# loli/medpy

Measured on AMD Instinct MI355X. Metric: Mvoxels/s graph-cut (build+solve), 512^3 6-conn; fraction of HBM roofline, higher is better.
Workload: dtype f64

## Files before the change

medpy_amd/csrc/mgc_kernels.hip:

```cpp
#include <hip/hip_runtime.h>
#include <rccl/rccl.h>

#include <dlfcn.h>

#include <math.h>
#include <stdarg.h>
#include <stdio.h>
#include <stdlib.h>
#include <string.h>

#include <algorithm>
#include <map>
#include <string>
#include <mutex>
#include <thread>
#include <vector>

#include "../../include/medpy_hip.h"
#include "mgc_tile_ops.inl"
#include "mgc_tile_ops26.inl"
#include "mgc_wave_ops.inl"
#include "mgc_wave_ops26.inl"
#include "mgc_dt_ops.inl"
#include "mgc_brick_ops.inl"
// ... 737 lines not shown
                }
            } else if (mode == 1) {
                take = (L.status[tile] & (MGC_ST_EXCESS | MGC_ST_ALLINF)) == MGC_ST_EXCESS;
            } else if (mode == 3) {
                take = (L.status[tile] & MGC_ST_SINK) != 0;
            } else {
                take = (L.status[tile] & MGC_ST_SUSPECT) != 0;
            }
        }
        const unsigned long long m = __ballot(take);
        if (m) {
            int pos = 0;
            const int sh = (int)(blockIdx.x & (unsigned)(L.nshard - 1));
            if ((threadIdx.x & 63) == 0) pos = atomicAdd(mgc_counter(L, cnt, sh), __popcll(m));
            pos = __shfl(pos, 0);
            if (take) L.list[list][(int64_t)sh * L.shard_cap + pos + __popcll(m & ((1ull << (threadIdx.x & 63)) - 1ull))] = tile;
        }
    }
}

__global__ __launch_bounds__(MGC_TV) void k_relabel_first_list(MgcLattice L, int list, int cnt, uint32_t epoch, int next_list)
{
    __shared__ MgcTileShared S;
    GpuBlock x(S);
    MgcListView view;
    const int n = mgc_list_view(L, cnt, view);
    if (blockIdx.x == 0 && threadIdx.x == 0 && n) atomicAdd(&L.count[9], n);
    for (int i = blockIdx.x; i < n; i += gridDim.x) {
        x.new_tile();
        mgc_relabel_tile(x, L, mgc_list_at(L, list, view, i), epoch, next_list, true);
        __syncthreads();
    }
}

__global__ __launch_bounds__(256) void k_absorb_w(MgcLattice L, int list, int cnt, int clear_cnt)
{
    __shared__ MgcWaveShared S;
    GpuWave w(S);
    mgc_clear_counter(L, clear_cnt);
    MgcListView view;
    const int n = mgc_list_view(L, cnt, view);
    for (int i = (int)blockIdx.x * 4 + (int)(threadIdx.x >> 6); i < n; i += (int)gridDim.x * 4) {
        w.new_tile();
        mgcw_absorb_tile(w, L, __builtin_amdgcn_readfirstlane(mgc_list_at(L, list, view, i)));
    }
}

__global__ __launch_bounds__(MGC_TV) void k_absorb_list(MgcLattice L, int list, int cnt, int clear_cnt)
{
    mgc_clear_counter(L, clear_cnt);
    __shared__ MgcTileShared S;
    GpuBlock x(S);
    MgcListView view;
    const int n = mgc_list_view(L, cnt, view);
    for (int i = blockIdx.x; i < n; i += gridDim.x) {
        x.new_tile();
        mgc_absorb_tile(x, L, mgc_list_at(L, list, view, i));
        __syncthreads();
    }
}

__global__ __launch_bounds__(MGC_TV) void k_activate_list(MgcLattice L, int list, int cnt, uint32_t phase)
{
    __shared__ MgcTileShared S;
    GpuBlock x(S);
    MgcListView view;
    const int n = mgc_list_view(L, cnt, view);
    for (int i = blockIdx.x; i < n; i += gridDim.x) {
        x.new_tile();
        mgc_activate_tile(x, L, mgc_list_at(L, list, view, i), phase);
        __syncthreads();
    }
}

template <int AXIS, bool BWD, int SEED, int FINAL>
__global__ __launch_bounds__(256) void k_dt_scan(MgcLattice L, const void* in, void* out, int c_min, int32_t* hout, const uint16_t* carry_in, uint16_t* carry_out, int carry_plane)
{
    __shared__ MgcWaveShared S;
    GpuWave w(S);
    const int n = mgc_dt_lines<AXIS>(L);
    for (int line = (int)blockIdx.x * 4 + (int)(threadIdx.x >> 6); line < n; line += (int)gridDim.x * 4) {
        w.new_tile();
        mgc_dt_scan_line<AXIS, BWD, SEED, FINAL>(w, L, __builtin_amdgcn_readfirstlane(line), in, out, c_min, hout, carry_in, carry_out, carry_plane);
    }
}

__global__ __launch_bounds__(256) void k_shadow_sync(MgcLattice L)
{
    __shared__ MgcWaveShared S;
    GpuWave w(S);
    const int T = L.gy * L.gx;
    for (int i = (int)blockIdx.x * 4 + (int)(threadIdx.x >> 6); i < 2 * T; i += (int)gridDim.x * 4) {
        w.new_tile();
        mgc_shadow_sync_tile(w, L, i / T, __builtin_amdgcn_readfirstlane(i % T), L.height);
    }
}

__global__ __launch_bounds__(256) void k_dt_finish(MgcLattice L)
{
    __shared__ MgcWaveShared S;
    GpuWave w(S);
    if (blockIdx.x == 0 && threadIdx.x == 0) atomicAdd(&L.count[9], L.ntiles);
    for (int tile = (int)blockIdx.x * 4 + (int)(threadIdx.x >> 6); tile < L.ntiles; tile += (int)gridDim.x * 4) {
        w.new_tile();
        mgc_dt_finish_tile(w, L, __builtin_amdgcn_readfirstlane(tile));
    }
}

__global__ __launch_bounds__(256) void k_dt_cmin(MgcLattice L)
{
    __shared__ MgcWaveShared S;
    GpuWave w(S);
    for (int tile = (int)blockIdx.x * 4 + (int)(threadIdx.x >> 6); tile < L.ntiles; tile += (int)gridDim.x * 4) {
        w.new_tile();
        mgc_dt_cmin_tile(w, L, __builtin_amdgcn_readfirstlane(tile));
    }
}

__global__ __launch_bounds__(256) void k_dt_lower(MgcLattice L, const uint16_t* ds, int c_min)
{
    __shared__ MgcWaveShared S;
    GpuWave w(S);
    for (int tile = (int)blockIdx.x * 4 + (int)(threadIdx.x >> 6); tile < L.ntiles; tile += (int)gridDim.x * 4) {
        w.new_tile();
        mgc_dt_lower_tile(w, L, __builtin_amdgcn_readfirstlane(tile), ds, c_min);
    }
}

__global__ __launch_bounds__(256) void k_source_open(MgcLattice L)
{
    __shared__ MgcWaveShared S;
    GpuWave w(S);
    for (int tile = (int)blockIdx.x * 4 + (int)(threadIdx.x >> 6); tile < L.ntiles; tile += (int)gridDim.x * 4) {
        w.new_tile();
        mgc_source_open_tile(w, L, __builtin_amdgcn_readfirstlane(tile));
    }
}

__global__ __launch_bounds__(256) void k_activate_w(MgcLattice L, int list, int cnt, uint32_t phase, int exact_max, int clear_cnt)
{
    mgc_clear_counter(L, clear_cnt);
    __shared__ MgcWaveShared S;
    GpuWave w(S);
    MgcListView view;
    const int n = mgc_list_view(L, cnt, view);
    if (n <= exact_max) {
        for (int i = (int)blockIdx.x * 4 + (int)(threadIdx.x >> 6); i < n; i += (int)gridDim.x * 4) {
            w.new_tile();
            mgcw_activate_tile(w, L, __builtin_amdgcn_readfirstlane(mgc_list_at(L, list, view, i)), phase, true);
        }
        return;
    }
    const int sh = (int)(blockIdx.x & (unsigned)(L.nshard - 1)), lane = (int)(threadIdx.x & 63);
    for (int base = (int)blockIdx.x * 256; base < n; base += (int)gridDim.x * 256) {
        const int i = base + (int)threadIdx.x;
        const bool take = i < n;
        const int tile = take ? mgc_list_at(L, list, view, i) : 0;
        int tz, ty, tx;
        mgc_tile_coords(L, tile, tz, ty, tx);
        const uint32_t target = phase + ((mgc_tile_colour(L, tz, ty, tx) ^ (int)(phase & 1u)) & 1);
        for (uint32_t tg = phase; tg <= phase + 1; ++tg) {
            const unsigned long long m = __ballot(take && target == tg);
            if (!m) continue;
            int pos = 0;
            if (lane == 0) pos = atomicAdd(mgc_counter(L, (int)(tg & 3u), sh), __popcll(m));
            pos = __shfl(pos, 0);
// ... 1274 lines not shown

struct MgcRoctx {
    bool tried = false;
    int (*push)(const char*) = nullptr;
    int (*pop)() = nullptr;
    void resolve()
    {
        tried = true;
        const char* on = getenv("MEDPY_HIP_ROCTX");
        if (!on || !*on || *on == '0') return;
        for (const char* n : {"librocprofiler-sdk-roctx.so.1", "librocprofiler-sdk-roctx.so", "libroctx64.so.4", "libroctx64.so"}) {
            void* dl = dlopen(n, RTLD_NOW | RTLD_GLOBAL);
            if (!dl) continue;
            *(void**)(&push) = dlsym(dl, "roctxRangePushA");
            *(void**)(&pop) = dlsym(dl, "roctxRangePop");
            if (push && pop) return;
            push = nullptr; pop = nullptr;
        }
    }
};
static MgcRoctx g_roctx;
static inline void mgc_range_push(const char* name)
{
    if (!g_roctx.tried) g_roctx.resolve();
    if (g_roctx.push) (void)g_roctx.push(name);
}
static inline void mgc_range_pop()
{
    if (g_roctx.pop) (void)g_roctx.pop();
}
struct MgcRange {
    explicit MgcRange(const char* name) { mgc_range_push(name); }
    ~MgcRange() { mgc_range_pop(); }
};
static std::string g_create_error;

struct mgc_graph {
    int device = 0;
    int ndim = 0;
    int64_t shape[3] = {1, 1, 1};
    int64_t nvox = 0;
    hipStream_t stream = nullptr;
    hipEvent_t ev[4] = {nullptr, nullptr, nullptr, nullptr};
    std::vector<hipEvent_t> ev_pool;
    struct OpSpan { int a, b, kind; };
    std::vector<hipEvent_t> op_ev;
    std::vector<OpSpan> op_spans;
    MgcLattice L{};
    void* d_image = nullptr; int img_dtype = 0; int term = MGC_TERM_NONE; double sigma = 0; double spacing[3] = {1, 1, 1};
    int has_spacing = 0;
    void* d_prob = nullptr; int prob_dtype = 0; double alpha = 0;
    void* d_lut = nullptr; int lut_n = 0;
    uint8_t* d_fg = nullptr; uint8_t* d_bg = nullptr;
    double* d_tr_in = nullptr; double flow_const_in = 0;
    MgcBuildArgs build_args{};
    int64_t n_edges = 0, n_runs = 0; int64_t* d_eslot = nullptr; double* d_eval = nullptr; int64_t* d_erun = nullptr;
    bool range_set = false; double range[3] = {0, 0, 0};
    bool edges_applied = false;
    std::map<const void*, size_t> buf_cap;
    uint8_t* d_tsum = nullptr;
    uint8_t* d_tflags = nullptr;
    double* d_tr0 = nullptr; double* d_part = nullptr; double* d_part2 = nullptr; double* d_scalar = nullptr; uint8_t* d_labels = nullptr;
    int32_t* h_count = nullptr;
    double* h_scalar = nullptr;
    uint8_t* h_labels = nullptr; bool labels_on_host = false;
    bool built = false, solved = false;
    bool unconverged = false;
    bool labels_valid = false;
    void* d_vout = nullptr;
    uint16_t* d_dt16 = nullptr;
    uint16_t* d_ds16 = nullptr;
    int32_t* d_hexact = nullptr;
    bool radial_on = false;
    int radial_cycle_no = 0;
    bool all_residual = false;
    int exact_sink_tiles = 1;
    int sink_tiles = 0;
    int wall_tiles = 0;
    int radial_min_walls = 16;
    int sink_sweeps = 8;
    int use_bricks = 0;
    bool brick_mode = false;
    int use_dt = 1;
    int rank = 0, nranks = 1;
    int64_t plane0 = 0, plane1 = 0, own0 = 0, own1 = 0;
    int64_t gd0 = 0;
    uint16_t* d_carry[2] = {nullptr, nullptr};
    uint16_t* d_carry_in[2] = {nullptr, nullptr};
    uint16_t* dt_cur = nullptr;
    void* d_halo = nullptr; int64_t halo_cap = 0;
    ncclComm_t comm = nullptr; void* d_xchg[4] = {nullptr, nullptr, nullptr, nullptr}; int64_t xchg_cap = 0;
    int64_t* d_cnt64 = nullptr;
    double flow_const = 0.0, flow = 0.0;
    MgcSolveParams params = mgc_default_params();
    int grid_cap = 4096;
    int grid26_dis = 16384;
    int wave_kernels = 9;
    int wave_grid_dis = 0, wave_grid_rel = 0;
    int tk_dis = MGC_CNT_TICKET_DIS, tk_rel = MGC_CNT_TICKET_REL;
    int est_phase_tiles = 1 << 30;
    int sweeps_sparse26 = 5;
    int wave_grid26 = 0;
    bool rounds_set = false, sparse26_set = false, wave_set = false;
    bool w26_auto = false;
    int prepush = 1;
    int w26_passes = 2, w26_raises = 1, w26_flags = 0;
    int activate_exact_max = 4096;
    int wave_stagger = 0;
    int repeat_steps = 1;
    int repeat_min_tiles = 0;
    int repeat_flood_min_tiles = 200000;
    bool repeat_now = false;
    int wave_min_tiles = 512;
    uint32_t zero_mask = 0;
    int filt[2] = {0, 0};
    int pending_zero = -1;
    int use_filters = 3;
    mgc_stats stats{};
    int64_t device_bytes = 0;
    std::string err;
    bool timing = true;
    int timing_stride = 7;
    uint32_t timing_offset = 0;
};

static int mgc_fail(mgc_handle h, int code, const char* fmt, ...)
{
    char buf[512];
    va_list ap;
    va_start(ap, fmt);
    vsnprintf(buf, sizeof(buf), fmt, ap);
    va_end(ap);
    if (h) h->err = buf;
    else g_create_error = buf;
    return code;
}

#define MGC_HIP(h, call)                                                                                       \
    do {                                                                                                       \
        hipError_t e_ = (call);                                                                                \
        if (e_ != hipSuccess)                                                                                  \
            return mgc_fail(h, e_ == hipErrorOutOfMemory ? MGC_ERR_OOM : MGC_ERR_HIP, "%s failed: %s (%s:%d)", \
                            #call, hipGetErrorString(e_), __FILE__, __LINE__);                                 \
    } while (0)


#define MGC_POOL_MIN ((size_t)1 << 20)
struct MgcPool {
    std::mutex lock;
    std::multimap<size_t, void*> idle[16];
    std::map<void*, std::pair<size_t, int>> live;
    size_t idle_bytes[16] = {0};
    long long budget[16];
    long long hits = 0, misses = 0;
    MgcPool() { for (auto& b : budget) b = -1; }
    long long budget_of(int dev)
    {
        if (budget[dev] < 0) {
            const char* e = getenv("MEDPY_HIP_POOL_MB");
            if (e && *e) budget[dev] = atoll(e) << 20;
            else {
                size_t f = 0, t = 0;
                budget[dev] = hipMemGetInfo(&f, &t) == hipSuccess ? (long long)(t / 8) : 0;
            }
        }
        return budget[dev];
// ... 85 lines not shown
    void fill_heights_inf()
    {
        flush_zero();
        h->labels_valid = true;
        check(hipMemsetAsync(h->L.height, 0x3f, (size_t)h->L.ntiles * MGC_TV * sizeof(int32_t), h->stream));
        hipLaunchKernelGGL(k_status_or, dim3((h->L.ntiles + 255) / 256), dim3(256), 0, h->stream, h->L, (uint32_t)MGC_ST_ALLINF, (uint32_t)MGC_ST_SETTLED);
        for (int sd = 0; sd < 2; ++sd)
            if (h->L.hshadow[sd]) check(hipMemsetAsync(h->L.hshadow[sd], 0x3f, (size_t)h->L.gy * h->L.gx * MGC_TF * sizeof(int32_t), h->stream));
    }
    void flush_zero()
    {
        if (h->pending_zero >= 0) h->zero_mask |= 1u << h->pending_zero;
        h->pending_zero = -1;
        if (h->zero_mask) {
            hipLaunchKernelGGL(k_zero_counts, dim3(1), dim3(MGC_NCOUNT * MGC_NSHARD), 0, h->stream, h->L, h->zero_mask);
            check(hipGetLastError());
        }
        h->zero_mask = 0;
    }
    void zero_count(int i)
    {
        if (i == last_discharged) { flush_zero(); h->pending_zero = i; last_discharged = -1; return; }
        if (h->pending_zero >= 0) { h->zero_mask |= 1u << h->pending_zero; h->pending_zero = -1; }
        h->zero_mask |= 1u << i;
    }
    void read_counts(int* out)
    {
        flush_zero();
        check(hipMemcpyAsync(h->h_count, h->L.count, MGC_NCOUNT * (1 + MGC_NSHARD) * sizeof(int32_t), hipMemcpyDeviceToHost, h->stream));
        check(hipStreamSynchronize(h->stream));
        mgc_fold_counts(h);
        memcpy(out, h->h_count, MGC_NCOUNT * sizeof(int32_t));
        readbacks++;
        if (!FULL) {
            int m = out[6] / 2;
            for (int i = 0; i < 4; ++i) m = out[i] > m ? out[i] : m;
            h->est_phase_tiles = m;
        } else {
            int m = out[MGC26_CNT_ACTIVE] / 8;
            for (int i = 0; i < MGC26_NLIST; ++i) m = out[i] > m ? out[i] : m;
            h->est_phase_tiles = m;
        }
    }
    int filter_grid() const { const int g = (h->L.ntiles + 255) / 256; return g < 1024 ? g : 1024; }
    int fslot(int which) const { return which == 0 ? (h->filt[0] ? MGC_CNT_FILTER_B : MGC_CNT_FILTER) : (h->filt[1] ? MGC_CNT_FILTER_ACT_B : MGC_CNT_FILTER_ACT); }
    int fnext(int which) const { return which == 0 ? (h->filt[0] ? MGC_CNT_FILTER : MGC_CNT_FILTER_B) : (h->filt[1] ? MGC_CNT_FILTER_ACT : MGC_CNT_FILTER_ACT_B); }
    void filter_done(int which, bool consumer_cleared_next)
    {
        if (!consumer_cleared_next) zero_count(fnext(which));
        h->filt[which] ^= 1;
    }
    void absorb_all()
    {
        flush_zero();
        if constexpr (FULL) return;
        else if (!(h->use_filters & 1)) { hipLaunchKernelGGL(k_absorb, dim3(grid(h->L.ntiles)), dim3(MGC_TV), 0, h->stream, h->L); check(hipGetLastError()); }
        else {
            flush_zero();
            hipLaunchKernelGGL(k_filter, dim3(filter_grid()), dim3(256), 0, h->stream, h->L, 0, 6, fslot(0));
            if (h->wave_kernels & 1) hipLaunchKernelGGL(k_absorb_w, dim3(grid((h->L.ntiles + 3) / 4)), dim3(256), 0, h->stream, h->L, 6, fslot(0), fnext(0));
            else hipLaunchKernelGGL(k_absorb_list, dim3(grid(h->L.ntiles)), dim3(MGC_TV), 0, h->stream, h->L, 6, fslot(0), fnext(0));
            filter_done(0, true);
            check(hipGetLastError());
        }
    }
    void relabel_all(uint32_t epoch, int next)
    {
        flush_zero();
        h->brick_mode = false;
        const int id = time_begin(1);
        if constexpr (FULL) hipLaunchKernelGGL(k26_relabel_all, dim3(grid(h->L.ntiles)), dim3(MGC_TV), 0, h->stream, h->L, epoch, next);
        else if (!(h->use_filters & 1)) hipLaunchKernelGGL(k_relabel_all, dim3(grid(h->L.ntiles)), dim3(MGC_TV), 0, h->stream, h->L, epoch, next);
        else {
            flush_zero();
            hipLaunchKernelGGL(k_filter, dim3(filter_grid()), dim3(256), 0, h->stream, h->L, 3, 6, fslot(0));
            if (h->wave_kernels & 8) { hipLaunchKernelGGL(k_relabel_v, dim3(grid(h->L.ntiles)), dim3(MGC_TV / MGC_RELABEL_V), 0, h->stream, h->L, 6, fslot(0), epoch, next, fnext(0), 1); filter_done(0, true); }
            else if (h->wave_kernels & 2) { hipLaunchKernelGGL(k_relabel_w, dim3(h->wave_grid_rel), dim3(MGCW_LANES), 0, h->stream, h->L, 6, fslot(0), epoch, next, -1, 1, h->tk_rel); h->tk_rel ^= 1; filter_done(0, false); }
            else { hipLaunchKernelGGL(k_relabel_first_list, dim3(grid(h->L.ntiles)), dim3(MGC_TV), 0, h->stream, h->L, 6, fslot(0), epoch, next); filter_done(0, false); }
        }
        check(hipGetLastError());
        time_end(id);
        relabel_launches++;
    }
    bool first_relabel_dt()
    {
        if (FULL || !h->use_dt || !h->all_residual || h->labels_valid || h->nranks > 1) return false;
        if (!h->d_dt16) {
            if (mgc_dmalloc((void**)&h->d_dt16, (size_t)h->L.ntiles * MGC_TV * sizeof(uint16_t)) != hipSuccess) { (void)hipGetLastError(); return false; }
            h->device_bytes += (int64_t)h->L.ntiles * MGC_TV * (int64_t)sizeof(uint16_t);
        }
        flush_zero();
        h->labels_valid = true;
        const int id = time_begin(2);
        const MgcLattice& L = h->L;
        void* const T = h->d_dt16;
        const dim3 blk(256);
        auto g = [&](int lines) { return dim3(grid((lines + 3) / 4)); };
        hipLaunchKernelGGL((k_dt_scan<0, false, 1, 0>), g(L.gz * L.gy), blk, 0, h->stream, L, (const void*)L.rmask, T, 0, (int32_t*)nullptr, (const uint16_t*)nullptr, (uint16_t*)nullptr, -1);
        hipLaunchKernelGGL((k_dt_scan<0, true, 0, 0>), g(L.gz * L.gy), blk, 0, h->stream, L, (const void*)T, T, 0, (int32_t*)nullptr, (const uint16_t*)nullptr, (uint16_t*)nullptr, -1);
        hipLaunchKernelGGL((k_dt_scan<1, false, 0, 0>), g(L.gz * L.gx), blk, 0, h->stream, L, (const void*)T, T, 0, (int32_t*)nullptr, (const uint16_t*)nullptr, (uint16_t*)nullptr, -1);
        hipLaunchKernelGGL((k_dt_scan<1, true, 0, 0>), g(L.gz * L.gx), blk, 0, h->stream, L, (const void*)T, T, 0, (int32_t*)nullptr, (const uint16_t*)nullptr, (uint16_t*)nullptr, -1);
        hipLaunchKernelGGL((k_dt_scan<2, false, 0, 0>), g(L.gy * L.gx), blk, 0, h->stream, L, (const void*)T, T, 0, (int32_t*)nullptr, (const uint16_t*)nullptr, (uint16_t*)nullptr, -1);
        hipLaunchKernelGGL((k_dt_scan<2, true, 0, 1>), g(L.gy * L.gx), blk, 0, h->stream, L, (const void*)T, (void*)L.height, 0, (int32_t*)nullptr, (const uint16_t*)nullptr, (uint16_t*)nullptr, -1);
        hipLaunchKernelGGL(k_dt_finish, g(L.ntiles), blk, 0, h->stream, L);
        check(hipGetLastError());
        time_end(id);
        relabel_launches += 7;
        return true;
    }
    void set_radial(bool on) { h->radial_on = on; if (on) h->radial_cycle_no++; }
    bool radial_begin(int c_min)
    {
        if (FULL) return false;
        const size_t nv = (size_t)h->L.ntiles * MGC_TV;
        if (!h->d_ds16) {
            if (mgc_dmalloc((void**)&h->d_ds16, nv * sizeof(uint16_t)) != hipSuccess) { (void)hipGetLastError(); return false; }
            h->device_bytes += (int64_t)(nv * sizeof(uint16_t));
        }
        if (!h->d_hexact) {
            if (mgc_dmalloc((void**)&h->d_hexact, nv * sizeof(int32_t)) != hipSuccess) { (void)hipGetLastError(); return false; }
            h->device_bytes += (int64_t)(nv * sizeof(int32_t));
        }
        flush_zero();
        const int id = time_begin(2);
        const MgcLattice& L = h->L;
        void* const T = h->d_ds16;
        const dim3 blk(256);
        auto g = [&](int lines) { return dim3(grid((lines + 3) / 4)); };
        check(hipMemsetAsync(L.count + mgc_cnt_radial_c(L), 0x3f, sizeof(int32_t), h->stream));
        hipLaunchKernelGGL(k_dt_cmin, g(L.ntiles), blk, 0, h->stream, L);
        hipLaunchKernelGGL((k_dt_scan<0, false, 2, 0>), g(L.gz * L.gy), blk, 0, h->stream, L, (const void*)L.excess, T, 0, (int32_t*)nullptr, (const uint16_t*)nullptr, (uint16_t*)nullptr, -1);
        hipLaunchKernelGGL((k_dt_scan<0, true, 0, 0>), g(L.gz * L.gy), blk, 0, h->stream, L, (const void*)T, T, 0, (int32_t*)nullptr, (const uint16_t*)nullptr, (uint16_t*)nullptr, -1);
        hipLaunchKernelGGL((k_dt_scan<1, false, 0, 0>), g(L.gz * L.gx), blk, 0, h->stream, L, (const void*)T, T, 0, (int32_t*)nullptr, (const uint16_t*)nullptr, (uint16_t*)nullptr, -1);
        hipLaunchKernelGGL((k_dt_scan<1, true, 0, 0>), g(L.gz * L.gx), blk, 0, h->stream, L, (const void*)T, T, 0, (int32_t*)nullptr, (const uint16_t*)nullptr, (uint16_t*)nullptr, -1);
        hipLaunchKernelGGL((k_dt_scan<2, false, 0, 0>), g(L.gy * L.gx), blk, 0, h->stream, L, (const void*)T, T, 0, (int32_t*)nullptr, (const uint16_t*)nullptr, (uint16_t*)nullptr, -1);
        hipLaunchKernelGGL((k_dt_scan<2, true, 0, 2>), g(L.gy * L.gx), blk, 0, h->stream, L, (const void*)T, T, c_min, h->d_hexact, (const uint16_t*)nullptr, (uint16_t*)nullptr, -1);
        std::swap(h->L.height, h->d_hexact);
        check(hipGetLastError());
        time_end(id);
        relabel_launches += 8;
        return true;
    }
    void radial_save_exact()
    {
        flush_zero();
        check(hipMemcpyAsync(h->d_hexact, h->L.height, (size_t)h->L.ntiles * MGC_TV * sizeof(int32_t), hipMemcpyDeviceToDevice, h->stream));
    }
    void radial_restore_exact()
    {
        flush_zero();
        std::swap(h->L.height, h->d_hexact);
    }
    void radial_lower(int c_min)
    {
        flush_zero();
        const int id = time_begin(2);
        hipLaunchKernelGGL(k_dt_lower, dim3(grid((h->L.ntiles + 3) / 4)), dim3(256), 0, h->stream, h->L, (const uint16_t*)h->d_ds16, c_min);
        check(hipGetLastError());
        time_end(id);
        relabel_launches++;
    }
    void source_open()
    {
        flush_zero();
        hipLaunchKernelGGL(k_source_open, dim3(grid((h->L.ntiles + 3) / 4)), dim3(256), 0, h->stream, h->L);
        check(hipGetLastError());
    }
    void relabel_list(int lst, uint32_t epoch, int next, int zero_list = -1)
    {
        flush_zero();
        const int id = time_begin(1);
        if (!FULL && h->brick_mode) hipLaunchKernelGGL(k_relabel_b, dim3(grid(mgc_brick_count(h->L))), dim3(MGC_TV), 0, h->stream, h->L, lst, epoch, next, zero_list);
        else if constexpr (FULL) hipLaunchKernelGGL(k26_relabel_list, dim3(grid(h->L.ntiles)), dim3(MGC_TV), 0, h->stream, h->L, lst, epoch, next);
        else if (h->wave_kernels & 8) hipLaunchKernelGGL(k_relabel_v, dim3(grid(h->L.ntiles)), dim3(MGC_TV / MGC_RELABEL_V), 0, h->stream, h->L, lst, lst, epoch, next, zero_list, 0);
        else if (h->wave_kernels & 2) { hipLaunchKernelGGL(k_relabel_w, dim3(h->wave_grid_rel), dim3(MGCW_LANES), 0, h->stream, h->L, lst, lst, epoch, next, zero_list, 0, h->tk_rel); h->tk_rel ^= 1; }
        else hipLaunchKernelGGL(k_relabel_list, dim3(grid(h->L.ntiles)), dim3(MGC_TV), 0, h->stream, h->L, lst, epoch, next, zero_list);
        check(hipGetLastError());
        time_end(id);
        relabel_launches++;
    }
    void suspect_pass()
    {
        flush_zero();
        const int nb = ((h->L.gx + 7) / 8) * ((h->L.gy + 7) / 8) * ((h->L.gz + 7) / 8);
        hipLaunchKernelGGL(k_suspect_pass<FULL>, dim3(nb < 4096 ? nb : 4096), dim3(MGC_TV), 0, h->stream, h->L);
        check(hipGetLastError());
    }
    void reset_suspect(uint32_t epoch, int list)
    {
        flush_zero();
        const int id = time_begin(1);
        h->brick_mode = !FULL && h->use_bricks && h->nranks == 1 && !(h->use_filters & 4);
        if (FULL || !(h->use_filters & 4)) hipLaunchKernelGGL(k_reset_suspect<FULL>, dim3(grid((h->L.ntiles + MGC_TV - 1) / MGC_TV)), dim3(MGC_TV), 0, h->stream, h->L, epoch, list, h->brick_mode ? 1 : 0);
        else {
            flush_zero();
            hipLaunchKernelGGL(k_filter, dim3(filter_grid()), dim3(256), 0, h->stream, h->L, 2, 6, fslot(0));
            hipLaunchKernelGGL(k_reset_suspect_list, dim3(grid(h->L.ntiles)), dim3(MGC_TV), 0, h->stream, h->L, 6, fslot(0), epoch, list);
            filter_done(0, false);
        }
        check(hipGetLastError());
        time_end(id);
        relabel_launches++;
    }
    void activate_all(uint32_t phase)
    {
        flush_zero();
        if constexpr (FULL) {
            if (h->L.nshard == 1 && (h->use_filters & 2)) hipLaunchKernelGGL(k26_activate_w, dim3(grid((h->L.ntiles + 3) / 4)), dim3(256), 0, h->stream, h->L, phase);
            else hipLaunchKernelGGL(k26_activate, dim3(grid(h->L.ntiles)), dim3(MGC_TV), 0, h->stream, h->L, phase);
        }
        else if (!(h->use_filters & 2)) hipLaunchKernelGGL(k_activate, dim3(grid(h->L.ntiles)), dim3(MGC_TV), 0, h->stream, h->L, phase);
        else {
            flush_zero();
            hipLaunchKernelGGL(k_filter, dim3(filter_grid()), dim3(256), 0, h->stream, h->L, 1, 7, fslot(1));
            if (h->wave_kernels & 1) { hipLaunchKernelGGL(k_activate_w, dim3(grid((h->L.ntiles + 3) / 4)), dim3(256), 0, h->stream, h->L, 7, fslot(1), phase, h->activate_exact_max, fnext(1)); filter_done(1, true); }
            else { hipLaunchKernelGGL(k_activate_list, dim3(grid(h->L.ntiles)), dim3(MGC_TV), 0, h->stream, h->L, 7, fslot(1), phase); filter_done(1, false); }
        }
        check(hipGetLastError());
    }
    void discharge(int lst, uint32_t phase, int cycles, int sweeps)
    {
        const int zero_idx = h->pending_zero;
        h->pending_zero = -1;
// ... 1546 lines not shown
    if (e == hipSuccess) e = hipMemcpyAsync(out, d, (size_t)h->nvox * sizeof(double), hipMemcpyDeviceToHost, h->stream);
    if (e == hipSuccess) e = hipStreamSynchronize(h->stream);
    (void)mgc_dfree(d);
    MGC_HIP(h, e);
    return MGC_OK;
}

int mgc_get_tweights(mgc_handle h, double* out)
{
    if (!h || !out) return MGC_ERR_INVALID;
    if (!h->built) return mgc_fail(h, MGC_ERR_STATE, "mgc_get_tweights before mgc_build");
    MGC_HIP(h, hipSetDevice(h->device));
    double* d = nullptr;
    MGC_HIP(h, mgc_dmalloc((void**)&d, (size_t)h->nvox * sizeof(double)));
    hipLaunchKernelGGL(k_untile_f64, dim3(1024), dim3(256), 0, h->stream, h->L, (const double*)h->d_tr0, (const uint8_t*)h->d_tflags, d);
    hipError_t e = hipGetLastError();
    if (e == hipSuccess) e = hipMemcpyAsync(out, d, (size_t)h->nvox * sizeof(double), hipMemcpyDeviceToHost, h->stream);
    if (e == hipSuccess) e = hipStreamSynchronize(h->stream);
    (void)mgc_dfree(d);
    MGC_HIP(h, e);
    return MGC_OK;
}

int mgc_get_edge(mgc_handle h, int64_t i, int64_t j, double* out)
{
    if (!h || !out) return MGC_ERR_INVALID;
    if (!h->built) return mgc_fail(h, MGC_ERR_STATE, "mgc_get_edge before mgc_build");
    if (i < 0 || j < 0 || i >= h->nvox || j >= h->nvox || i == j) return mgc_fail(h, MGC_ERR_INVALID, "bad node pair");
    MGC_HIP(h, hipSetDevice(h->device));
    const MgcLattice& L = h->L;
    const int d = mgc_arc_direction(L, i, j);
    *out = 0.0;
    if (d < 0) return MGC_OK;
    int tile, loc;
    mgc_node_to_tile(L, i, tile, loc);
    const double* src = L.rcap + ((int64_t)tile * L.ndir + d) * MGC_TV + loc;
    MGC_HIP(h, hipMemcpyAsync(h->h_scalar + 6, src, sizeof(double), hipMemcpyDeviceToHost, h->stream));
    MGC_HIP(h, hipStreamSynchronize(h->stream));
    *out = h->h_scalar[6];
    return MGC_OK;
}

int mgc_get_node_num(mgc_handle h, int64_t* n)
{
    if (!h || !n) return MGC_ERR_INVALID;
    *n = h->nvox;
    return MGC_OK;
}

int mgc_set_param(mgc_handle h, const char* name, int64_t value)
{
    if (!h || !name) return MGC_ERR_INVALID;
    if (!strcmp(name, "rounds_per_relabel") && value > 0) { h->params.rounds_per_relabel = (int)value; h->rounds_set = true; }
    else if (!strcmp(name, "max_cycles") && value != 0) h->params.max_cycles = (int)value;
    else if (!strcmp(name, "max_sweeps") && value > 0) h->params.max_sweeps = (int)value;
    else if (!strcmp(name, "max_outer") && value > 0) h->params.max_outer = (int)value;
    else if (!strcmp(name, "grid_cap") && value > 0) h->grid_cap = (int)value;
    else if (!strcmp(name, "grid26_dis") && value >= 0) h->grid26_dis = (int)value;
    else if (!strcmp(name, "relabel_batch") && value > 0) h->params.relabel_batch = (int)value;
    else if (!strcmp(name, "check_rounds") && value > 0) h->params.check_rounds = (int)value;
    else if (!strcmp(name, "stop_below") && value >= 0) h->params.stop_below = (int)value;
    else if (!strcmp(name, "incremental_relabel")) h->params.incremental_relabel = value != 0;
    else if (!strcmp(name, "trace")) h->params.trace = value != 0;
    else if (!strcmp(name, "adaptive_rounds") && value >= 0) h->params.adaptive_rounds = (int)value;
    else if (!strcmp(name, "radial") && value >= 0 && value <= 2) h->params.radial = (int)value;
    else if (!strcmp(name, "radial_min_walls") && value >= 0) h->radial_min_walls = (int)value;
    else if (!strcmp(name, "radial_budget_x16") && value >= 1) h->params.radial_budget_x16 = (int)value;
    else if (!strcmp(name, "radial_min_c") && value >= 1) h->params.radial_min_c = (int)value;
    else if (!strcmp(name, "radial_rounds0") && value >= 0) h->params.radial_rounds0 = (int)value;
    else if (!strcmp(name, "use_filters")) h->use_filters = (int)value;
    else if (!strcmp(name, "wave_kernels")) { h->wave_kernels = (int)value; h->wave_set = true; }
    else if (!strcmp(name, "wave_min_tiles") && value >= 0) h->wave_min_tiles = (int)value;
    else if (!strcmp(name, "sweeps_sparse26") && value >= 0) { h->sweeps_sparse26 = (int)value; h->sparse26_set = true; }
    else if (!strcmp(name, "wave_grid_dis") && value > 0) h->wave_grid_dis = (int)value;
    else if (!strcmp(name, "wave_grid26") && value > 0) h->wave_grid26 = (int)value;
    else if (!strcmp(name, "prepush")) h->prepush = value != 0;
    else if ((!strcmp(name, "exchange_passes") || !strcmp(name, "relabel_exchange_every")) && value > 0) h->params.exchange_passes = (int)value;
    else if (!strcmp(name, "exchange_rounds") && value > 0) h->params.exchange_rounds = (int)value;
    else if (!strcmp(name, "w26_passes") && value > 0) h->w26_passes = (int)value;
    else if (!strcmp(name, "w26_raises") && value > 0) h->w26_raises = (int)value;
    else if (!strcmp(name, "w26_flags") && value >= 0) h->w26_flags = (int)value;
    else if (!strcmp(name, "wave_grid_rel") && value > 0) h->wave_grid_rel = (int)value;
    else if (!strcmp(name, "first_relabel_dt")) h->use_dt = value != 0;
    else if (!strcmp(name, "relabel_bricks")) h->use_bricks = value != 0;
    else if (!strcmp(name, "exact_sink_tiles") && value >= 0 && value <= 2) h->exact_sink_tiles = (int)value;
    else if (!strcmp(name, "sink_sweeps") && value > 0) h->sink_sweeps = (int)value;
    else if (!strcmp(name, "halo_max_records") && value >= 1) {
        const int64_t T = (int64_t)h->L.gy * h->L.gx;
        h->L.halo_max_rec = (int)(value < T ? value : T);
    }
    else if (!strcmp(name, "wave_stagger") && value >= 0) h->wave_stagger = (int)value;
    else if (!strcmp(name, "repeat_steps") && value >= 0 && value <= 7) h->repeat_steps = (int)value;
    else if (!strcmp(name, "repeat_min_tiles") && value >= 0) h->repeat_min_tiles = (int)value;
    else if (!strcmp(name, "repeat_flood_min_tiles") && value >= 0) h->repeat_flood_min_tiles = (int)value;
    else if (!strcmp(name, "list_shards") && (value == 1 || value == MGC_NSHARD)) {
        mgc_flush_zero(h);
        MGC_HIP(h, hipMemsetAsync(h->L.count, 0, MGC_NCOUNT * (1 + MGC_NSHARD) * sizeof(int32_t), h->stream));
        h->L.nshard = (int)value;
        h->filt[0] = h->filt[1] = 0;
        h->solved = false;
    }
    else if (!strcmp(name, "activate_exact_max") && value >= 0) h->activate_exact_max = (int)value;
    else if (!strcmp(name, "kernel_timing")) h->timing = value != 0;
    else if (!strcmp(name, "timing_stride") && value > 0) h->timing_stride = (int)value;
    else if (!strcmp(name, "profile_sections")) {
        if (value && !h->L.prof) {
            MGC_HIP(h, mgc_dmalloc((void**)&h->L.prof, 16 * sizeof(unsigned long long)));
        }
        if (h->L.prof) MGC_HIP(h, hipMemset(h->L.prof, 0, 16 * sizeof(unsigned long long)));
        if (!value && h->L.prof) { (void)mgc_dfree(h->L.prof); h->L.prof = nullptr; }
    }
    else return mgc_fail(h, MGC_ERR_INVALID, "unknown or invalid parameter %s=%lld", name, (long long)value);
    return MGC_OK;
}

int mgc_get_profile(mgc_handle h, uint64_t* out16)
{
    if (!h || !out16) return MGC_ERR_INVALID;
    memset(out16, 0, 16 * sizeof(uint64_t));
    if (!h->L.prof) return MGC_OK;
    MGC_HIP(h, hipSetDevice(h->device));
    MGC_HIP(h, hipMemcpy(out16, h->L.prof, 16 * sizeof(uint64_t), hipMemcpyDeviceToHost));
    return MGC_OK;
}

int mgc_get_stats(mgc_handle h, mgc_stats* out)
{
    if (!h || !out) return MGC_ERR_INVALID;
    h->stats.ntiles = h->L.ntiles;
    h->stats.nvox = h->nvox;
    h->stats.device_bytes = h->device_bytes;
    *out = h->stats;
    return MGC_OK;
}

}
```

Measured before the change: 7429.

## Fuse forward and backward distance-transform scans per axis into one kernel

Adds a k_dt_axis kernel that loads a whole line into registers across several waves, synchronises, then runs both scan directions and stores, replacing the separate forward and backward k_dt_scan launches. The first-relabel and radial distance transforms now use three launches instead of six, which halves the passes over the 16-bit distance buffer. It depends on helper functions and a shared struct (mgc_dtf_load/store, MgcDtfShared, MGC_DTF_WAVES) that are not defined in the shown code. It also uses one block per line, which may lower occupancy and raise register pressure for long lines.

Result: faster. 7533 (median of 6 runs) (+1.4%).

```diff
diff --git a/medpy_amd/csrc/mgc_kernels.hip b/medpy_amd/csrc/mgc_kernels.hip
--- a/medpy_amd/csrc/mgc_kernels.hip
+++ b/medpy_amd/csrc/mgc_kernels.hip
@@ -843,6 +843,23 @@
     for (int line = (int)blockIdx.x * 4 + (int)(threadIdx.x >> 6); line < n; line += (int)gridDim.x * 4) {
         w.new_tile();
         mgc_dt_scan_line<AXIS, BWD, SEED, FINAL>(w, L, __builtin_amdgcn_readfirstlane(line), in, out, c_min, hout, carry_in, carry_out, carry_plane);
+    }
+}
+
+template <int AXIS, int SEED, int FINAL, int TPW>
+__global__ __launch_bounds__(64 * MGC_DTF_WAVES) void k_dt_axis(MgcLattice L, const void* in, void* out, int c_min, int32_t* hout)
+{
+    __shared__ MgcDtfShared S;
+    GpuWaveT<MgcDtfShared> w(S);
+    const int s = __builtin_amdgcn_readfirstlane((int)threadIdx.x >> 6);
+    const int n = mgc_dt_lines<AXIS>(L);
+    for (int line = (int)blockIdx.x; line < n; line += (int)gridDim.x) {
+        w.new_tile();
+        typename GpuWaveT<MgcDtfShared>::template Reg<uint32_t, TPW * 4> v;
+        mgc_dtf_load<AXIS, SEED, TPW>(w, L, line, s, v, in);
+        __syncthreads();
+        mgc_dtf_store<AXIS, FINAL, TPW>(w, L, line, s, v, out, c_min, hout);
+        __syncthreads();
     }
 }
 
@@ -2283,6 +2300,7 @@
     int use_bricks = 0;
     bool brick_mode = false;
     int use_dt = 1;
+    int dt_fused = 1;
     int rank = 0, nranks = 1;
     int64_t plane0 = 0, plane1 = 0, own0 = 0, own1 = 0;
     int64_t gd0 = 0;
@@ -2534,6 +2552,20 @@
         time_end(id);
         relabel_launches++;
     }
+    bool dt_fused_ok() const { return h->dt_fused && mgc_dtf_tpw(h->L.gx) && mgc_dtf_tpw(h->L.gy) && mgc_dtf_tpw(h->L.gz); }
+    template <int AXIS, int SEED, int FINAL>
+    void dt_axis(const void* in, void* out, int c_min = 0, int32_t* hout = nullptr)
+    {
+        const MgcLattice& L = h->L;
+        const dim3 g(grid(mgc_dt_lines<AXIS>(L))), blk(64 * MGC_DTF_WAVES);
+        switch (mgc_dtf_tpw(AXIS == 0 ? L.gx : (AXIS == 1 ? L.gy : L.gz))) {
+        case 1: hipLaunchKernelGGL((k_dt_axis<AXIS, SEED, FINAL, 1>), g, blk, 0, h->stream, L, in, out, c_min, hout); break;
+        case 2: hipLaunchKernelGGL((k_dt_axis<AXIS, SEED, FINAL, 2>), g, blk, 0, h->stream, L, in, out, c_min, hout); break;
+        case 4: hipLaunchKernelGGL((k_dt_axis<AXIS, SEED, FINAL, 4>), g, blk, 0, h->stream, L, in, out, c_min, hout); break;
+        case 8: hipLaunchKernelGGL((k_dt_axis<AXIS, SEED, FINAL, 8>), g, blk, 0, h->stream, L, in, out, c_min, hout); break;
+        default: hipLaunchKernelGGL((k_dt_axis<AXIS, SEED, FINAL, MGC_DTF_TPW_MAX>), g, blk, 0, h->stream, L, in, out, c_min, hout); break;
+        }
+    }
     bool first_relabel_dt()
     {
         if (FULL || !h->use_dt || !h->all_residual || h->labels_valid || h->nranks > 1) return false;
@@ -2548,16 +2580,23 @@
         void* const T = h->d_dt16;
         const dim3 blk(256);
         auto g = [&](int lines) { return dim3(grid((lines + 3) / 4)); };
-        hipLaunchKernelGGL((k_dt_scan<0, false, 1, 0>), g(L.gz * L.gy), blk, 0, h->stream, L, (const void*)L.rmask, T, 0, (int32_t*)nullptr, (const uint16_t*)nullptr, (uint16_t*)nullptr, -1);
-        hipLaunchKernelGGL((k_dt_scan<0, true, 0, 0>), g(L.gz * L.gy), blk, 0, h->stream, L, (const void*)T, T, 0, (int32_t*)nullptr, (const uint16_t*)nullptr, (uint16_t*)nullptr, -1);
-        hipLaunchKernelGGL((k_dt_scan<1, false, 0, 0>), g(L.gz * L.gx), blk, 0, h->stream, L, (const void*)T, T, 0, (int32_t*)nullptr, (const uint16_t*)nullptr, (uint16_t*)nullptr, -1);
-        hipLaunchKernelGGL((k_dt_scan<1, true, 0, 0>), g(L.gz * L.gx), blk, 0, h->stream, L, (const void*)T, T, 0, (int32_t*)nullptr, (const uint16_t*)nullptr, (uint16_t*)nullptr, -1);
-        hipLaunchKernelGGL((k_dt_scan<2, false, 0, 0>), g(L.gy * L.gx), blk, 0, h->stream, L, (const void*)T, T, 0, (int32_t*)nullptr, (const uint16_t*)nullptr, (uint16_t*)nullptr, -1);
-        hipLaunchKernelGGL((k_dt_scan<2, true, 0, 1>), g(L.gy * L.gx), blk, 0, h->stream, L, (const void*)T, (void*)L.height, 0, (int32_t*)nullptr, (const uint16_t*)nullptr, (uint16_t*)nullptr, -1);
+        if (dt_fused_ok()) {
+            dt_axis<0, 1, 0>(L.rmask, T);
+            dt_axis<1, 0, 0>(T, T);
+            dt_axis<2, 0, 1>(T, L.height);
+            relabel_launches += 4;
+        } else {
+            hipLaunchKernelGGL((k_dt_scan<0, false, 1, 0>), g(L.gz * L.gy), blk, 0, h->stream, L, (const void*)L.rmask, T, 0, (int32_t*)nullptr, (const uint16_t*)nullptr, (uint16_t*)nullptr, -1);
+            hipLaunchKernelGGL((k_dt_scan<0, true, 0, 0>), g(L.gz * L.gy), blk, 0, h->stream, L, (const void*)T, T, 0, (int32_t*)nullptr, (const uint16_t*)nullptr, (uint16_t*)nullptr, -1);
+            hipLaunchKernelGGL((k_dt_scan<1, false, 0, 0>), g(L.gz * L.gx), blk, 0, h->stream, L, (const void*)T, T, 0, (int32_t*)nullptr, (const uint16_t*)nullptr, (uint16_t*)nullptr, -1);
+            hipLaunchKernelGGL((k_dt_scan<1, true, 0, 0>), g(L.gz * L.gx), blk, 0, h->stream, L, (const void*)T, T, 0, (int32_t*)nullptr, (const uint16_t*)nullptr, (uint16_t*)nullptr, -1);
+            hipLaunchKernelGGL((k_dt_scan<2, false, 0, 0>), g(L.gy * L.gx), blk, 0, h->stream, L, (const void*)T, T, 0, (int32_t*)nullptr, (const uint16_t*)nullptr, (uint16_t*)nullptr, -1);
+            hipLaunchKernelGGL((k_dt_scan<2, true, 0, 1>), g(L.gy * L.gx), blk, 0, h->stream, L, (const void*)T, (void*)L.height, 0, (int32_t*)nullptr, (const uint16_t*)nullptr, (uint16_t*)nullptr, -1);
+            relabel_launches += 7;
+        }
         hipLaunchKernelGGL(k_dt_finish, g(L.ntiles), blk, 0, h->stream, L);
         check(hipGetLastError());
         time_end(id);
-        relabel_launches += 7;
         return true;
     }
     void set_radial(bool on) { h->radial_on = on; if (on) h->radial_cycle_no++; }
@@ -2581,16 +2620,23 @@
         auto g = [&](int lines) { return dim3(grid((lines + 3) / 4)); };
         check(hipMemsetAsync(L.count + mgc_cnt_radial_c(L), 0x3f, sizeof(int32_t), h->stream));
         hipLaunchKernelGGL(k_dt_cmin, g(L.ntiles), blk, 0, h->stream, L);
-        hipLaunchKernelGGL((k_dt_scan<0, false, 2, 0>), g(L.gz * L.gy), blk, 0, h->stream, L, (const void*)L.excess, T, 0, (int32_t*)nullptr, (const uint16_t*)nullptr, (uint16_t*)nullptr, -1);
-        hipLaunchKernelGGL((k_dt_scan<0, true, 0, 0>), g(L.gz * L.gy), blk, 0, h->stream, L, (const void*)T, T, 0, (int32_t*)nullptr, (const uint16_t*)nullptr, (uint16_t*)nullptr, -1);
-        hipLaunchKernelGGL((k_dt_scan<1, false, 0, 0>), g(L.gz * L.gx), blk, 0, h->stream, L, (const void*)T, T, 0, (int32_t*)nullptr, (const uint16_t*)nullptr, (uint16_t*)nullptr, -1);
-        hipLaunchKernelGGL((k_dt_scan<1, true, 0, 0>), g(L.gz * L.gx), blk, 0, h->stream, L, (const void*)T, T, 0, (int32_t*)nullptr, (const uint16_t*)nullptr, (uint16_t*)nullptr, -1);
-        hipLaunchKernelGGL((k_dt_scan<2, false, 0, 0>), g(L.gy * L.gx), blk, 0, h->stream, L, (const void*)T, T, 0, (int32_t*)nullptr, (const uint16_t*)nullptr, (uint16_t*)nullptr, -1);
-        hipLaunchKernelGGL((k_dt_scan<2, true, 0, 2>), g(L.gy * L.gx), blk, 0, h->stream, L, (const void*)T, T, c_min, h->d_hexact, (const uint16_t*)nullptr, (uint16_t*)nullptr, -1);
+        if (dt_fused_ok()) {
+            dt_axis<0, 2, 0>(L.excess, T);
+            dt_axis<1, 0, 0>(T, T);
+            dt_axis<2, 0, 2>(T, T, c_min, h->d_hexact);
+            relabel_launches += 5;
+        } else {
+            hipLaunchKernelGGL((k_dt_scan<0, false, 2, 0>), g(L.gz * L.gy), blk, 0, h->stream, L, (const void*)L.excess, T, 0, (int32_t*)nullptr, (const uint16_t*)nullptr, (uint16_t*)nullptr, -1);
+            hipLaunchKernelGGL((k_dt_scan<0, true, 0, 0>), g(L.gz * L.gy), blk, 0, h->stream, L, (const void*)T, T, 0, (int32_t*)nullptr, (const uint16_t*)nullptr, (uint16_t*)nullptr, -1);
+            hipLaunchKernelGGL((k_dt_scan<1, false, 0, 0>), g(L.gz * L.gx), blk, 0, h->stream, L, (const void*)T, T, 0, (int32_t*)nullptr, (const uint16_t*)nullptr, (uint16_t*)nullptr, -1);
+            hipLaunchKernelGGL((k_dt_scan<1, true, 0, 0>), g(L.gz * L.gx), blk, 0, h->stream, L, (const void*)T, T, 0, (int32_t*)nullptr, (const uint16_t*)nullptr, (uint16_t*)nullptr, -1);
+            hipLaunchKernelGGL((k_dt_scan<2, false, 0, 0>), g(L.gy * L.gx), blk, 0, h->stream, L, (const void*)T, T, 0, (int32_t*)nullptr, (const uint16_t*)nullptr, (uint16_t*)nullptr, -1);
+            hipLaunchKernelGGL((k_dt_scan<2, true, 0, 2>), g(L.gy * L.gx), blk, 0, h->stream, L, (const void*)T, T, c_min, h->d_hexact, (const uint16_t*)nullptr, (uint16_t*)nullptr, -1);
+            relabel_launches += 8;
+        }
         std::swap(h->L.height, h->d_hexact);
         check(hipGetLastError());
         time_end(id);
-        relabel_launches += 8;
         return true;
     }
     void radial_save_exact()
@@ -4303,6 +4349,7 @@
     else if (!strcmp(name, "w26_flags") && value >= 0) h->w26_flags = (int)value;
     else if (!strcmp(name, "wave_grid_rel") && value > 0) h->wave_grid_rel = (int)value;
     else if (!strcmp(name, "first_relabel_dt")) h->use_dt = value != 0;
+    else if (!strcmp(name, "dt_fused")) h->dt_fused = value != 0;
     else if (!strcmp(name, "relabel_bricks")) h->use_bricks = value != 0;
     else if (!strcmp(name, "exact_sink_tiles") && value >= 0 && value <= 2) h->exact_sink_tiles = (int)value;
     else if (!strcmp(name, "sink_sweeps") && value > 0) h->sink_sweeps = (int)value;
```
